# TongkunGuan/CCD

Hardware: AMD Instinct MI355X
Metric: images/sec (32x128 crops, 2 views) CCD-ViT-Small pretrain step (higher is better)
Workload: dtype bf16; 1 GPU; CCD_pretrain_vit_small bf16, bs=256/GPU, 2 views 32x128, out_dim=65536, drop_path 0.1, dataset-mask branch (pseudo-epoch 1), synthetic batch in HBM; global_batch=256, parallelism=dp1

## Files before the change

### ccd_amd/csrc/abi_impl.h

```cpp
#pragma once

#include "../../include/ccd_hip.h"
#include "kernels/common.h"
#include "kernels/gemm.h"
#include "kernels/gemm256.h"
#include "kernels/gemm_row384.h"
#include "kernels/mlp_fused.h"
#include "kernels/rowgemm.h"
#include "kernels/mlp_bwd.h"
#include "kernels/rowproj.h"
#include "kernels/attention_fwd.h"
#include "kernels/attention_probs.h"
#include "kernels/attention_bwd.h"
#include "kernels/attention_bwd1.h"
#include "kernels/gemm_tn384.h"
#include "kernels/layernorm.h"
#include "kernels/charmap.h"
#include "kernels/cluster.h"
#include "kernels/ssim.h"
#include "kernels/segmetric.h"
#include "kernels/textscore.h"
#include "kernels/ctc.h"
#include "kernels/ctc_beam.h"
#include "kernels/nrtr_beam.h"
// ... 959 lines not shown
    CCD_CHECK(ccd::aug_spatial_smem(height, width) <= 160 * 1024, CCD_ESHAPE);
    CCD_CHECK(std3[0] > 0.f && std3[1] > 0.f && std3[2] > 0.f, CCD_EINVAL);
    if (batch == 0) return CCD_OK;
    CCD_LAUNCH(ccd::augment_spatial_kernel, dim3(2 * batch), dim3(256), (int)ccd::aug_spatial_smem(height, width), stream, img, params,
               staged_ws, height, width, overlay, overlay_layers);
    CCD_LAUNCH(ccd::augment_views_kernel, dim3((height * width + 255) / 256, batch), dim3(256), 0, stream, img, staged_ws, theta,
               out, batch, height, width, mean3[0], mean3[1], mean3[2], 1.0f / std3[0], 1.0f / std3[1], 1.0f / std3[2], params, warp_maps,
               warp_count);
    return ccd_rt_last_error();
}
int ccd_warp_idmap(const uint8_t* src, const float* theta, int theta_stride, uint8_t* dst, int images, void* stream) {
    CCD_CHECK(src && theta && dst && images >= 0 && theta_stride >= 6, CCD_EINVAL);
    if (images == 0) return CCD_OK;
    CCD_LAUNCH(ccd::warp_idmap_kernel, dim3(ccd::CM_PIX / 256, images), dim3(256), 0, stream, src, theta, theta_stride,
               dst, images);
    return ccd_rt_last_error();
}
int ccd_region_stats(const uint8_t* idmap, uint8_t* tok_plane, float* tok_coef, uint8_t* present, int views,
                     void* stream) {
    CCD_CHECK(idmap && tok_plane && tok_coef && present && views >= 0, CCD_EINVAL);
    if (views == 0) return CCD_OK;
    CCD_LAUNCH(ccd::region_stats_kernel, dim3(views), dim3(256), 0, stream, idmap, tok_plane, tok_coef, present, views);
    return ccd_rt_last_error();
}
int ccd_select_scan(const uint8_t* present, int batch, int* nsel, int* offset, int* total, uint8_t* new_index,
                    void* stream) {
    CCD_CHECK(present && nsel && offset && total && new_index && batch > 0, CCD_EINVAL);
    CCD_LAUNCH(ccd::select_scan_kernel, dim3(1), dim3(256), 0, stream, present, batch, nsel, offset, total, new_index);
    return ccd_rt_last_error();
}
int ccd_region_pool_fwd(const ccd_bf16* feat, const uint8_t* tok_plane, const float* tok_coef, const int* nsel,
                        const int* offset, const int* total, ccd_bf16* rows, int batch, int E, void* stream) {
    CCD_CHECK(feat && tok_plane && tok_coef && nsel && offset && total && rows && batch > 0 && E > 0, CCD_EINVAL);
    const size_t smem = (size_t)ccd::CM_PLANES * E * 4;
    CCD_CHECK(smem <= 120 * 1024 && E % 2 == 0, CCD_ESHAPE);
    CCD_LAUNCH(ccd::region_pool_fwd_kernel, dim3(2 * batch), dim3(256), smem, stream, feat, tok_plane, tok_coef, nsel,
               offset, total, rows, batch, E);
    return ccd_rt_last_error();
}
int ccd_region_pool_bwd(const ccd_bf16* d_rows, const uint8_t* tok_plane, const float* tok_coef, const int* nsel,
                        const int* offset, const int* total, ccd_bf16* d_feat, int batch, int E, void* stream) {
    CCD_CHECK(d_rows && tok_plane && tok_coef && nsel && offset && total && d_feat && batch > 0 && E > 0, CCD_EINVAL);
    CCD_CHECK(E % 8 == 0, CCD_ESHAPE);
    CCD_LAUNCH(ccd::region_pool_bwd_kernel, dim3(2 * batch), dim3(256), 0, stream, d_rows, tok_plane, tok_coef, nsel,
               offset, total, d_feat, batch, E);
    return ccd_rt_last_error();
}
int ccd_idmap_to_planes(const uint8_t* idmap, float* planes, int images, void* stream) {
    CCD_CHECK(idmap && planes && images >= 0, CCD_EINVAL);
    if (images == 0) return CCD_OK;
    const long n = (long)images * ccd::CM_PLANES * ccd::CM_PIX;
    CCD_LAUNCH(ccd::idmap_to_planes_kernel, dim3((unsigned)((n + 255) / 256)), dim3(256), 0, stream, idmap, planes,
               (long)images);
    return ccd_rt_last_error();
}
int ccd_planes_to_idmap(const float* planes, uint8_t* idmap, int images, void* stream) {
    CCD_CHECK(idmap && planes && images >= 0, CCD_EINVAL);
    if (images == 0) return CCD_OK;
    const long n = (long)images * ccd::CM_PIX;
    CCD_LAUNCH(ccd::planes_to_idmap_kernel, dim3((unsigned)((n + 255) / 256)), dim3(256), 0, stream, planes, idmap,
               (long)images);
    return ccd_rt_last_error();
}

int ccd_dbscan_label(const float* mask, uint8_t* idmap, int images, void* stream) {
    CCD_CHECK(images >= 0, CCD_EINVAL);
    if (images == 0) return CCD_OK;
    CCD_CHECK(mask && idmap, CCD_EINVAL);
    CCD_LAUNCH(ccd::dbscan_label_kernel, dim3(images), dim3(256), 0, stream, mask, idmap, images);
    return ccd_rt_last_error();
}
int ccd_region_boxes(const float* mask, int* boxes, int* count, int images, void* stream) {
    CCD_CHECK(images >= 0, CCD_EINVAL);
    if (images == 0) return CCD_OK;
    CCD_CHECK(mask && boxes && count, CCD_EINVAL);
    CCD_LAUNCH(ccd::region_boxes_kernel, dim3(images), dim3(256), 0, stream, mask, boxes, count, images);
    return ccd_rt_last_error();
// ... 431 lines not shown
int ccd_nrtr_beam_reorder(ccd_bf16* cache, const int* parent, int layers, int batch, int beam, int positions, int D, int step, void* stream) {
    CCD_CHECK(layers >= 0 && batch >= 0 && step >= 0, CCD_EINVAL);
    CCD_CHECK(beam >= 1 && beam <= ccd::NRTR_MAX_BEAM && positions >= 1 && step < positions && D >= 8 && D % 8 == 0, CCD_ESHAPE);
    if (layers == 0 || batch == 0) return CCD_OK;
    CCD_CHECK(cache && parent && CCD_ALIGNED16(cache), CCD_EINVAL);
    const long total = (long)layers * batch * (step + 1) * (D / 4);
    CCD_CHECK((total + 255) / 256 <= 0x7fffffffL, CCD_ESHAPE);
    CCD_LAUNCH(ccd::nrtr_beam_reorder_kernel, dim3((unsigned)((total + 255) / 256)), dim3(256), 0, stream,
               reinterpret_cast<ccd::bf16_t*>(cache), parent, layers, batch, beam, positions, D, step, total);
    return ccd_rt_last_error();
}

int ccd_l2norm_fwd(const ccd_bf16* x, ccd_bf16* y, float* inv, int max_rows, const int* d_rows, int rows_mul, int D,
                   void* stream) {
    CCD_CHECK(x && y && inv && max_rows >= 0, CCD_EINVAL);
    if (max_rows == 0) return CCD_OK;
    CCD_CHECK(D > 0 && D <= 64 * ccd::HD_MAX_PER_LANE, CCD_ESHAPE);
    CCD_LAUNCH(ccd::l2norm_fwd_kernel, dim3((max_rows + 3) / 4), dim3(256), 0, stream, x, y, inv, max_rows, d_rows,
               rows_mul, D);
    return ccd_rt_last_error();
}
int ccd_l2norm_bwd(const ccd_bf16* x, const float* inv, const ccd_bf16* dy, ccd_bf16* dx, int max_rows,
                   const int* d_rows, int rows_mul, int D, void* stream) {
    CCD_CHECK(x && inv && dy && dx && max_rows >= 0, CCD_EINVAL);
    if (max_rows == 0) return CCD_OK;
    CCD_CHECK(D > 0 && D <= 64 * ccd::HD_MAX_PER_LANE, CCD_ESHAPE);
    CCD_LAUNCH(ccd::l2norm_bwd_kernel, dim3((max_rows + 3) / 4), dim3(256), 0, stream, x, inv, dy, dx, max_rows, d_rows,
               rows_mul, D);
    return ccd_rt_last_error();
}
int ccd_weightnorm_fwd(const float* v, const float* g, ccd_bf16* w, ccd_bf16* w_t, float* inv, int K, int D,
                       void* stream) {
    CCD_CHECK(v && g && w && inv && K > 0 && D > 0, CCD_EINVAL);
    const size_t smem = (size_t)ccd::WN_ROWS * (D + 1) * 4;
    CCD_CHECK(smem <= 128 * 1024 && D % 4 == 0 && D <= 256 * ccd::WN_MAX_V4 && K % 2 == 0, CCD_ESHAPE);
    CCD_LAUNCH(ccd::weightnorm_fwd_kernel, dim3((K + ccd::WN_ROWS - 1) / ccd::WN_ROWS), dim3(256), smem, stream, v, g, w, w_t, inv, K, D);
    return ccd_rt_last_error();
}
int ccd_weightnorm_bwd(const float* v, const float* g, const float* inv, const float* dw, float* dv, float* dg, int K,
                       int D, void* stream) {
    CCD_CHECK(v && g && inv && dw && dv && K > 0 && D > 0, CCD_EINVAL);
    CCD_LAUNCH(ccd::weightnorm_bwd_kernel, dim3((K + 3) / 4), dim3(256), 0, stream, v, g, inv, dw, dv, dg, K, D);
    return ccd_rt_last_error();
}

int ccd_dino_loss_fwd(const float* s_logits, const float* t_logits, const float* center, int K, const int* d_m,
                      int max_rows, float student_temp, float teacher_temp, float* stats, float* loss_out,
                      void* stream) {
    CCD_CHECK(s_logits && t_logits && center && d_m && stats && loss_out, CCD_EINVAL);
    CCD_CHECK(K > 0 && K % 4 == 0 && max_rows > 0 && student_temp > 0 && teacher_temp > 0, CCD_ESHAPE);
    CCD_LAUNCH(ccd::dino_loss_fwd_kernel, dim3(max_rows), dim3(256), 0, stream, s_logits, t_logits, center, K, d_m,
               max_rows, 1.0f / student_temp, 1.0f / teacher_temp, stats, loss_out);
    return ccd_rt_last_error();
}
int ccd_dino_loss_bwd(const float* s_logits, const float* t_logits, const float* center, int K, const int* d_m,
                      int max_rows, float student_temp, float teacher_temp, const float* stats, float grad_scale,
                      const float* d_grad_scale, ccd_bf16* d_logits, void* stream) {
    CCD_CHECK(s_logits && t_logits && center && d_m && stats && d_logits, CCD_EINVAL);
    CCD_CHECK(K > 0 && K % 4 == 0 && max_rows > 0 && student_temp > 0 && teacher_temp > 0, CCD_ESHAPE);
    CCD_LAUNCH(ccd::dino_loss_bwd_kernel, dim3(max_rows), dim3(256), 0, stream, s_logits, t_logits, center, K, d_m,
               max_rows, 1.0f / student_temp, 1.0f / teacher_temp, stats, grad_scale, d_grad_scale, d_logits);
    return ccd_rt_last_error();
}
static int ccd_head_loss_splits(int K) {
    if (K <= 0 || K % 512 != 0) return 0;
    const int chunks_total = K / 64;
    for (int cs = 64; cs >= 8; cs -= 8)
        if (chunks_total % cs == 0) return cs;
// ... 730 lines not shown
```

### ccd_amd/csrc/kernels/charmap.h

```cpp
#pragma once

namespace ccd {

constexpr int CM_H = 32, CM_W = 128, CM_PIX = CM_H * CM_W, CM_PLANES = 26, CM_MIN_AREA = 30;
constexpr unsigned char CM_BG = 255;

__device__ __forceinline__ void cm_components(int* label, int* changed) {
    const int t = threadIdx.x;
    for (;;) {
        if (t == 0) *changed = 0;
        __syncthreads();
        for (int i = t; i < CM_PIX; i += 256) {
            const int li = label[i];
            if (li < 0) continue;
            const int y = i >> 7, x = i & 127;
            int best = li;
#pragma unroll
            for (int dy = -1; dy <= 1; ++dy)
#pragma unroll
                for (int dx = -1; dx <= 1; ++dx) {
                    const int yy = y + dy, xx = x + dx;
                    if (yy < 0 || yy >= CM_H || xx < 0 || xx >= CM_W) continue;
                    const int ln = label[yy * CM_W + xx];
                    if (ln >= 0 && ln < best) best = ln;
// ... 181 lines not shown
                                                          unsigned char* __restrict__ new_index) {
    __shared__ int part[256];
    const int t = threadIdx.x;
    const int per = (batch + 255) / 256;
    int local = 0;
    for (int k = 0; k < per; ++k) {
        const int b = t * per + k;
        if (b >= batch) break;
        int c = 0;
        for (int j = 0; j < CM_PLANES; ++j) c += present[(long)b * CM_PLANES + j];
        c = c < 3 ? 3 : (c > 26 ? 26 : c);
        const int n = c + 1 < CM_PLANES ? c + 1 : CM_PLANES;
        nsel[b] = n;
        local += n;
        for (int j = 0; j < CM_PLANES; ++j) new_index[(long)b * CM_PLANES + j] = j <= c ? 1 : 0;
    }
    part[t] = local;
    __syncthreads();
    if (t == 0) {
        int run = 0;
        for (int k = 0; k < 256; ++k) { const int v = part[k]; part[k] = run; run += v; }
        total[0] = run;
    }
    __syncthreads();
    int run = part[t];
    for (int k = 0; k < per; ++k) {
        const int b = t * per + k;
        if (b >= batch) break;
        offset[b] = run;
        run += nsel[b];
    }
}

__global__ __launch_bounds__(256) void region_pool_fwd_kernel(const bf16_t* __restrict__ feat,
                                                              const unsigned char* __restrict__ tok_plane,
                                                              const float* __restrict__ tok_coef,
                                                              const int* __restrict__ nsel, const int* __restrict__ offset,
                                                              const int* __restrict__ total, bf16_t* __restrict__ rows,
                                                              int batch, int E) {
    float* acc = reinterpret_cast<float*>(dynamic_smem());
    __shared__ unsigned char s_plane[256 * 4];
    __shared__ float s_coef[256 * 4];
    const int view = blockIdx.x, b = view % batch, half = view / batch;
    const int t = threadIdx.x;
#pragma unroll
    for (int s = 0; s < 4; ++s) {
        s_plane[4 * t + s] = tok_plane[((long)view * 256 + t) * 4 + s];
        s_coef[4 * t + s] = tok_coef[((long)view * 256 + t) * 4 + s];
    }
    const int n = nsel[b];
    for (int i = t; i < n * E; i += 256) acc[i] = 0.0f;
    __syncthreads();
    const bf16_t* f = feat + (long)view * 256 * E;
    for (int e2 = t; 2 * e2 < E; e2 += 256) {
        for (int tok0 = 0; tok0 < 256; tok0 += 8) {
            unsigned wv[8];
#pragma unroll
            for (int u = 0; u < 8; ++u) wv[u] = *reinterpret_cast<const unsigned*>(f + (long)(tok0 + u) * E + 2 * e2);
#pragma unroll
            for (int u = 0; u < 8; ++u) {
                const int tok = tok0 + u;
                if (s_plane[4 * tok] == CM_BG) continue;
                const float x0 = bf_lo(wv[u]), x1 = bf_hi(wv[u]);
#pragma unroll
                for (int s = 0; s < 4; ++s) {
                    const int p = s_plane[4 * tok + s];
                    if (p < n) {
                        const float cf = s_coef[4 * tok + s];
                        acc[p * E + 2 * e2] += cf * x0;
                        acc[p * E + 2 * e2 + 1] += cf * x1;
                    }
                }
            }
        }
    }
    __syncthreads();
    bf16_t* out = rows + ((long)half * total[0] + offset[b]) * E;
    for (int i = t; i < n * E; i += 256) out[i] = f2bf(acc[i]);
}

__global__ __launch_bounds__(256) void region_pool_bwd_kernel(const bf16_t* __restrict__ d_rows,
                                                              const unsigned char* __restrict__ tok_plane,
                                                              const float* __restrict__ tok_coef,
                                                              const int* __restrict__ nsel, const int* __restrict__ offset,
                                                              const int* __restrict__ total, bf16_t* __restrict__ d_feat,
                                                              int batch, int E) {
    const int view = blockIdx.x, b = view % batch, half = view / batch;
    const int n = nsel[b];
    const bf16_t* base = d_rows + ((long)half * total[0] + offset[b]) * E;
    bf16_t* out = d_feat + (long)view * 256 * E;
    const int e8 = E >> 3;
    for (int i = threadIdx.x; i < 256 * e8; i += 256) {
        const int tok = i / e8, c = i % e8;
        float a[8] = {0.f, 0.f, 0.f, 0.f, 0.f, 0.f, 0.f, 0.f};
#pragma unroll
        for (int s = 0; s < 4; ++s) {
            const int p = tok_plane[((long)view * 256 + tok) * 4 + s];
            if (p < n) {
                const float coef = tok_coef[((long)view * 256 + tok) * 4 + s];
                float v[8];
                unpack8(*reinterpret_cast<const u32x4*>(base + (long)p * E + c * 8), v);
#pragma unroll
                for (int k = 0; k < 8; ++k) a[k] += v[k] * coef;
            }
        }
        *reinterpret_cast<u32x4*>(out + (long)tok * E + c * 8) = pack8(a);
    }
}

__global__ void idmap_to_planes_kernel(const unsigned char* __restrict__ idmap, float* __restrict__ planes, long images) {
    const long i = (long)blockIdx.x * blockDim.x + threadIdx.x;
    if (i >= images * CM_PLANES * CM_PIX) return;
    const long img = i / (CM_PLANES * CM_PIX);
    const int plane = (int)((i / CM_PIX) % CM_PLANES), pix = (int)(i % CM_PIX);
    planes[i] = idmap[img * CM_PIX + pix] == plane ? 1.0f : 0.0f;
}
__global__ void planes_to_idmap_kernel(const float* __restrict__ planes, unsigned char* __restrict__ idmap, long images) {
    const long i = (long)blockIdx.x * blockDim.x + threadIdx.x;
    if (i >= images * CM_PIX) return;
    const long img = i / CM_PIX;
    const int pix = (int)(i % CM_PIX);
    int id = CM_BG;
    for (int p = CM_PLANES - 1; p >= 0; --p)
        if (planes[(img * CM_PLANES + p) * CM_PIX + pix] > 0.0f) id = p;
    idmap[i] = (unsigned char)id;
}

}
```

### ccd_amd/csrc/kernels/embed.h

```cpp
#pragma once

namespace ccd {

constexpr int PE_PATCH = 4, PE_K = 48, PE_GW = 32, PE_GH = 8;

__global__ __launch_bounds__(128) void patch_embed_fwd_kernel(const float* __restrict__ img, const float* __restrict__ w,
                                                              const float* __restrict__ bias,
                                                              const float* __restrict__ pos, float* __restrict__ out,
                                                              int E) {
    __shared__ float px[3][PE_PATCH][PE_GW * PE_PATCH];
    const int view = blockIdx.x / PE_GH, py = blockIdx.x % PE_GH;
    const float* src = img + (long)view * 3 * 32 * 128;
    for (int i = threadIdx.x; i < 3 * 4 * 128; i += blockDim.x) {
        const int c = i / 512, r = (i / 128) % 4, x = i % 128;
        px[c][r][x] = src[(long)c * 4096 + (py * 4 + r) * 128 + x];
    }
    __syncthreads();
    for (int e = threadIdx.x; e < E; e += blockDim.x) {
        float wr[PE_K];
#pragma unroll
        for (int k = 0; k < PE_K; ++k) wr[k] = w[(long)e * PE_K + k];
        const float b = bias[e];
        for (int tx = 0; tx < PE_GW; ++tx) {
            float acc = 0.f;
// ... 152 lines not shown
#pragma unroll
                for (int k = 0; k < 8; ++k) acc[k] += v[k];
            }
        }
        for (; r < r1; r += rln) {
            float v[8];
            unpack8(*reinterpret_cast<const u32x4*>(x + (long)r * ld + col), v);
#pragma unroll
            for (int k = 0; k < 8; ++k) acc[k] += v[k];
        }
    }
#pragma unroll
    for (int k = 0; k < 8; ++k) red[threadIdx.x][k] = acc[k];
    __syncthreads();
    if ((int)threadIdx.x < 8 * cgn) {
        const int c_local = threadIdx.x, g = c_local >> 3, k = c_local & 7;
        const int c = blockIdx.x * cgn * 8 + c_local;
        if (c < N) {
            float s = 0.f;
            for (int j = 0; j < rln; ++j) s += red[j * cgn + g][k];
            atomicAdd(out + c, s);
        }
    }
}

struct MirrorDesc {
    const float* src;
    bf16_t* dst;
    bf16_t* dst_t;
    int rows, cols;
    int tile_begin;
};
constexpr int MIRROR_TILE = 64;
__global__ __launch_bounds__(256) void mirror_bf16_kernel(const MirrorDesc* __restrict__ descs, int ndesc) {
    __shared__ float tile[MIRROR_TILE][MIRROR_TILE + 1];
    int d = 0;
    while (d + 1 < ndesc && descs[d + 1].tile_begin <= (int)blockIdx.x) ++d;
    const MirrorDesc m = descs[d];
    const int tiles_c = (m.cols + MIRROR_TILE - 1) / MIRROR_TILE;
    const int tl = blockIdx.x - m.tile_begin, tr = tl / tiles_c, tc = tl % tiles_c;
    const int lx = threadIdx.x & 63, ly = threadIdx.x >> 6;
    for (int i = ly; i < MIRROR_TILE; i += 4) {
        const int r = tr * MIRROR_TILE + i, c = tc * MIRROR_TILE + lx;
        float v = 0.f;
        if (r < m.rows && c < m.cols) {
            v = m.src[(long)r * m.cols + c];
            if (m.dst) m.dst[(long)r * m.cols + c] = f2bf(v);
        }
        tile[i][lx] = v;
    }
    __syncthreads();
    if (m.dst_t) {
        const int rp = threadIdx.x & 31, cy = threadIdx.x >> 5;
        const int r = tr * MIRROR_TILE + 2 * rp;
        const bool pairs = (m.rows & 1) == 0;
        for (int i = cy; i < MIRROR_TILE; i += 8) {
            const int c = tc * MIRROR_TILE + i;
            if (c >= m.cols) break;
            bf16_t* o = m.dst_t + (long)c * m.rows + r;
            if (pairs && r + 1 < m.rows) *reinterpret_cast<unsigned*>(o) = pack_bf2(tile[2 * rp][i], tile[2 * rp + 1][i]);
            else {
                if (r < m.rows) o[0] = f2bf(tile[2 * rp][i]);
                if (r + 1 < m.rows) o[1] = f2bf(tile[2 * rp + 1][i]);
            }
        }
    }
}

__global__ __launch_bounds__(256) void scale_cast_rows_kernel(const float* __restrict__ src, bf16_t* __restrict__ dst,
                                                              const float* __restrict__ rowscale, int rows_per_sample,
                                                              long rows, int E) {
    const int e4 = E >> 2;
    const long i = (long)blockIdx.x * 256 + threadIdx.x;
    if (i >= rows * e4) return;
    const long r = i / e4;
    const int c = (int)(i % e4) * 4;
    const float s = rowscale ? rowscale[r / rows_per_sample] : 1.0f;
    const f32x4v v = *reinterpret_cast<const f32x4v*>(src + r * E + c);
    u32x2 o;
    o.x = pack_bf2(v.x * s, v.y * s);
    o.y = pack_bf2(v.z * s, v.w * s);
    *reinterpret_cast<u32x2*>(dst + r * E + c) = o;
}

__global__ void cast_bf16_kernel(const float* __restrict__ src, bf16_t* __restrict__ dst, long n) {
    const long i = ((long)blockIdx.x * blockDim.x + threadIdx.x) * 4;
    if (i + 3 < n) {
        const f32x4v v = *reinterpret_cast<const f32x4v*>(src + i);
        u32x2 o;
        o.x = pack_bf2(v.x, v.y);
        o.y = pack_bf2(v.z, v.w);
        *reinterpret_cast<u32x2*>(dst + i) = o;
    } else {
        for (long k = i; k < n; ++k) dst[k] = f2bf(src[k]);
    }
}

// ... 2 lines not shown
```

### ccd_amd/csrc/kernels/head.h

```cpp
#pragma once

namespace ccd {

constexpr int HD_MAX_PER_LANE = 8;

__global__ __launch_bounds__(256) void l2norm_fwd_kernel(const bf16_t* __restrict__ x, bf16_t* __restrict__ y,
                                                         float* __restrict__ inv_out, int max_rows,
                                                         const int* __restrict__ d_rows, int rows_mul, int D) {
    const int lane = threadIdx.x & 63;
    const int row = blockIdx.x * 4 + (threadIdx.x >> 6);
    const int rows = d_rows ? d_rows[0] * rows_mul : max_rows;
    if (row >= rows || row >= max_rows) return;
    float v[HD_MAX_PER_LANE];
    float s = 0.f;
#pragma unroll
    for (int i = 0; i < HD_MAX_PER_LANE; ++i) {
        const int c = lane + 64 * i;
        v[i] = c < D ? bf2f(x[(long)row * D + c]) : 0.f;
        s += v[i] * v[i];
    }
    const float nrm = sqrtf(wave_sum(s));
    const float inv = 1.0f / fmaxf(nrm, 1e-12f);
#pragma unroll
    for (int i = 0; i < HD_MAX_PER_LANE; ++i) {
// ... 2 lines not shown
    }
    if (lane == 0) inv_out[row] = inv;
}
__global__ __launch_bounds__(256) void l2norm_bwd_kernel(const bf16_t* __restrict__ x, const float* __restrict__ inv_in,
                                                         const bf16_t* __restrict__ dy, bf16_t* __restrict__ dx,
                                                         int max_rows, const int* __restrict__ d_rows, int rows_mul,
                                                         int D) {
    const int lane = threadIdx.x & 63;
    const int row = blockIdx.x * 4 + (threadIdx.x >> 6);
    const int rows = d_rows ? d_rows[0] * rows_mul : max_rows;
    if (row >= rows || row >= max_rows) return;
    const float inv = inv_in[row];
    float yv[HD_MAX_PER_LANE], dv[HD_MAX_PER_LANE];
    float dot = 0.f;
#pragma unroll
    for (int i = 0; i < HD_MAX_PER_LANE; ++i) {
        const int c = lane + 64 * i;
        yv[i] = c < D ? bf2f(x[(long)row * D + c]) * inv : 0.f;
        dv[i] = c < D ? bf2f(dy[(long)row * D + c]) : 0.f;
        dot += yv[i] * dv[i];
    }
    dot = wave_sum(dot);
#pragma unroll
    for (int i = 0; i < HD_MAX_PER_LANE; ++i) {
        const int c = lane + 64 * i;
        if (c < D) dx[(long)row * D + c] = f2bf(inv * (dv[i] - yv[i] * dot));
    }
}

constexpr int WN_ROWS = 64, WN_MAX_V4 = 4;
__global__ __launch_bounds__(256) void weightnorm_fwd_kernel(const float* __restrict__ v, const float* __restrict__ g,
                                                             bf16_t* __restrict__ w, bf16_t* __restrict__ w_t,
                                                             float* __restrict__ inv_out, int K, int D) {
    float* tile = reinterpret_cast<float*>(dynamic_smem());
    const int lane = threadIdx.x & 63, wv = threadIdx.x >> 6;
    const int k0 = blockIdx.x * WN_ROWS;
    const int d4 = D >> 2;
    for (int r = wv; r < WN_ROWS; r += 4) {
        const int k = k0 + r;
        if (k >= K) break;
        const f32x4v* row = reinterpret_cast<const f32x4v*>(v + (long)k * D);
        f32x4v x[WN_MAX_V4];
        float s = 0.f;
#pragma unroll
        for (int j = 0; j < WN_MAX_V4; ++j) {
            const int c4 = lane + 64 * j;
            x[j] = c4 < d4 ? row[c4] : f32x4v{0.f, 0.f, 0.f, 0.f};
            s += x[j].x * x[j].x + x[j].y * x[j].y + x[j].z * x[j].z + x[j].w * x[j].w;
        }
        const float inv = 1.0f / sqrtf(wave_sum(s));
        const float sc = g[k] * inv;
#pragma unroll
        for (int j = 0; j < WN_MAX_V4; ++j) {
            const int c4 = lane + 64 * j;
            if (c4 < d4) {
                const float a0 = x[j].x * sc, a1 = x[j].y * sc, a2 = x[j].z * sc, a3 = x[j].w * sc;
                u32x2 o;
                o.x = pack_bf2(a0, a1); o.y = pack_bf2(a2, a3);
                *reinterpret_cast<u32x2*>(w + (long)k * D + 4 * c4) = o;
                float* t = tile + r * (D + 1) + 4 * c4;
                t[0] = a0; t[1] = a1; t[2] = a2; t[3] = a3;
            }
        }
        if (lane == 0) inv_out[k] = inv;
    }
    __syncthreads();
    if (w_t) {
        const int kp = threadIdx.x & 31;
        for (int c = threadIdx.x >> 5; c < D; c += 8)
            if (k0 + 2 * kp + 1 < K)
                *reinterpret_cast<unsigned*>(w_t + (long)c * K + k0 + 2 * kp) =
                    pack_bf2(tile[(2 * kp) * (D + 1) + c], tile[(2 * kp + 1) * (D + 1) + c]);
    }
}
__global__ __launch_bounds__(256) void weightnorm_bwd_kernel(const float* __restrict__ v, const float* __restrict__ g,
                                                             const float* __restrict__ inv_in,
                                                             const float* __restrict__ dw, float* __restrict__ dv,
                                                             float* __restrict__ dg, int K, int D) {
    const int lane = threadIdx.x & 63;
    const int k = blockIdx.x * 4 + (threadIdx.x >> 6);
    if (k >= K) return;
    const float inv = inv_in[k], gk = g[k];
    float dot = 0.f;
    for (int c = lane; c < D; c += 64) dot += dw[(long)k * D + c] * v[(long)k * D + c] * inv;
    dot = wave_sum(dot);
    for (int c = lane; c < D; c += 64) {
        const float vh = v[(long)k * D + c] * inv;
        dv[(long)k * D + c] = gk * inv * (dw[(long)k * D + c] - vh * dot);
    }
    if (dg && lane == 0) dg[k] = dot;
}

}
```

### ccd_amd/engine.py

```python
from __future__ import annotations

import math

import os

import torch

from . import ops

BF16, F32 = torch.bfloat16, torch.float32


class VitSpec:
    def __init__(self, embed_dim, depth, heads, taps, patch=4, eps=1e-6, drop_path_rate=0.0):
        self.E, self.depth, self.heads, self.taps, self.patch, self.eps = embed_dim, depth, heads, tuple(taps), patch, eps
        self.dpr = [x.item() for x in torch.linspace(0, drop_path_rate, depth)]
        self._keep = {}

    def keep_probs(self, device):
        if device not in self._keep:
            self._keep[device] = torch.tensor([1.0 - d for d in self.dpr], dtype=F32, device=device)
        return self._keep[device]


# ... 414 lines not shown
    @staticmethod
    def backward(ctx, d_tokens, *d_taps):
        m = ctx.module
        cast = lambda t: None if t is None else t.contiguous().to(BF16)
        backbone_backward(m.arena, m.arena_prefix, m.spec, ctx.saved, cast(d_tokens), [cast(t) for t in d_taps],
                          m.resample, m.grad_ready_hook)
        ctx.saved = None
        return None, None, None, None


class Selection:

    def __init__(self, idmap, batch):
        self.idmap, self.batch = idmap, batch
        self.tok_plane, self.tok_coef, self.present = ops.region_stats(idmap)
        self.nsel, self.offset, self.total, self.new_index = ops.select_scan(self.present, batch)
        self.max_rows = 2 * 26 * batch
        self._m = None

    @property
    def M(self):
        if self._m is None:
            self._m = int(self.total.item())
        return self._m

    def dense(self):
        return ops.idmap_to_planes(self.idmap)


class RegionPoolFn(torch.autograd.Function):
    @staticmethod
    def forward(ctx, tokens, sel: Selection):
        E = tokens.shape[-1]
        rows = torch.zeros((sel.max_rows, E), dtype=BF16, device=tokens.device)
        ops.region_pool_fwd(tokens.contiguous(), sel.tok_plane, sel.tok_coef, sel.nsel, sel.offset, sel.total, rows,
                            sel.batch)
        ctx.sel, ctx.shape = sel, tokens.shape
        return rows

    @staticmethod
    def backward(ctx, d_rows):
        sel = ctx.sel
        d_feat = torch.empty(ctx.shape, dtype=BF16, device=d_rows.device)
        ops.region_pool_bwd(d_rows.contiguous().to(BF16), sel.tok_plane, sel.tok_coef, sel.nsel, sel.offset, sel.total,
                            d_feat, sel.batch)
        return d_feat, None


class LazyLogits:

    def __init__(self, zn, w, d_total, rows_mul):
        self.zn, self.w, self.d_total, self.rows_mul = zn, w, d_total, rows_mul
        self.stub = None
        self._tensor = None

    @property
    def shape(self):
        return torch.Size((self.zn.shape[0], self.w.shape[0]))

    @property
    def device(self):
        return self.zn.device

    def detach(self):
        return self

    def tensor(self):
# ... 210 lines not shown
```

### ccd_amd/ops.py

```python
from __future__ import annotations

import ctypes
import math

import numpy as np
import torch

from . import _lib

EPI_BF16, EPI_GELU, EPI_RESID, EPI_F32, EPI_ATOMIC, EPI_DGELU = range(6)
BF16, F32 = torch.bfloat16, torch.float32
_EPI_NAMES = ("bf16", "gelu", "resid", "f32", "atomic", "dgelu")


class KernelTimer:

    def __init__(self, only=None):
        self.records = []
        self.only = only

    def span(self, key, flops, nbytes=0.0):
        if self.only is not None and key not in self.only:
            return None
        e0, e1 = torch.cuda.Event(enable_timing=True), torch.cuda.Event(enable_timing=True)
# ... 443 lines not shown
    _call("ccd_augment_views", img, params, theta, out, staged, B, H, W, m3, s3, overlay, int(layers), warp_maps, int(maps))
    return out


def warp_idmap(src, theta):
    assert src.dtype == U8 and src.is_contiguous() and theta.dtype == F32 and theta.is_contiguous()
    out = torch.empty_like(src)
    _call("ccd_warp_idmap", src, theta, theta.stride(0), out, src.shape[0])
    return out


def region_stats(idmap):
    views = idmap.shape[0]
    dev = idmap.device
    tok_plane = torch.empty((views, 256, 4), dtype=U8, device=dev)
    tok_coef = torch.empty((views, 256, 4), dtype=F32, device=dev)
    present = torch.empty((views, 26), dtype=U8, device=dev)
    _call("ccd_region_stats", idmap, tok_plane, tok_coef, present, views)
    return tok_plane, tok_coef, present


def select_scan(present, batch):
    dev = present.device
    nsel = torch.empty(batch, dtype=I32, device=dev)
    offset = torch.empty(batch, dtype=I32, device=dev)
    total = torch.empty(1, dtype=I32, device=dev)
    new_index = torch.empty((batch, 26), dtype=U8, device=dev)
    _call("ccd_select_scan", present, batch, nsel, offset, total, new_index)
    return nsel, offset, total, new_index


def region_pool_fwd(feat, tok_plane, tok_coef, nsel, offset, total, rows, batch):
    E = feat.shape[-1]
    _call("ccd_region_pool_fwd", feat, tok_plane, tok_coef, nsel, offset, total, rows, batch, E)
    return rows


def region_pool_bwd(d_rows, tok_plane, tok_coef, nsel, offset, total, d_feat, batch):
    E = d_feat.shape[-1]
    _call("ccd_region_pool_bwd", d_rows, tok_plane, tok_coef, nsel, offset, total, d_feat, batch, E)
    return d_feat


def idmap_to_planes(idmap):
    out = torch.empty((idmap.shape[0], 26, 32, 128), dtype=F32, device=idmap.device)
    _call("ccd_idmap_to_planes", idmap, out, idmap.shape[0])
    return out


def planes_to_idmap(planes):
    planes = planes.contiguous().float()
    out = torch.empty((planes.shape[0], 32, 128), dtype=U8, device=planes.device)
    _call("ccd_planes_to_idmap", planes, out, planes.shape[0])
    return out


def dbscan_label(mask):
    assert mask.dtype == F32 and mask.is_contiguous() and tuple(mask.shape[1:]) == (32, 128)
    out = torch.empty(mask.shape, dtype=U8, device=mask.device)
    _call("ccd_dbscan_label", mask, out, mask.shape[0])
    return out


def region_boxes(mask):
    assert mask.dtype == F32 and mask.is_contiguous() and tuple(mask.shape[1:]) == (32, 128)
    boxes = torch.empty((mask.shape[0], 26, 4), dtype=I32, device=mask.device)
# ... 1307 lines not shown
```

Baseline: 5554 images/sec.

## Rework region pooling, weightnorm, and mirror kernels for parallelism and vectorized access

Region pool forward moves from one 256-thread block per view to many 64-thread blocks, each owning a channel slab. The new version double-buffers token chunks through LDS, zero-fills the unused output rows inside the kernel, and drops the separate torch.zeros memset. Region pool backward splits each view across four blocks and stages plane and coefficient data in shared memory. The weightnorm forward/backward and the fp32-to-bf16 mirror/transpose kernels switch to vectorized 128-bit loads and stores, with bf16 LDS tiles using swizzled or padded layouts. These changes target low occupancy and narrow memory accesses, at the cost of more complex indexing and a cap of 27 region planes per view in forward.

```diff
diff --git a/ccd_amd/csrc/abi_impl.h b/ccd_amd/csrc/abi_impl.h
--- a/ccd_amd/csrc/abi_impl.h
+++ b/ccd_amd/csrc/abi_impl.h
@@ -1015,17 +1015,20 @@
 int ccd_region_pool_fwd(const ccd_bf16* feat, const uint8_t* tok_plane, const float* tok_coef, const int* nsel,
                         const int* offset, const int* total, ccd_bf16* rows, int batch, int E, void* stream) {
     CCD_CHECK(feat && tok_plane && tok_coef && nsel && offset && total && rows && batch > 0 && E > 0, CCD_EINVAL);
-    const size_t smem = (size_t)ccd::CM_PLANES * E * 4;
-    CCD_CHECK(smem <= 120 * 1024 && E % 2 == 0, CCD_ESHAPE);
-    CCD_LAUNCH(ccd::region_pool_fwd_kernel, dim3(2 * batch), dim3(256), smem, stream, feat, tok_plane, tok_coef, nsel,
-               offset, total, rows, batch, E);
+    CCD_CHECK(E % 8 == 0, CCD_ESHAPE);
+    if (E % 128 == 0)
+        CCD_LAUNCH(ccd::region_pool_fwd_kernel<16>, dim3(2 * batch * (E / 128)), dim3(64), 0, stream, feat, tok_plane, tok_coef, nsel,
+                   offset, total, rows, batch, E);
+    else
+        CCD_LAUNCH(ccd::region_pool_fwd_kernel<8>, dim3(2 * batch * ((E + 63) / 64)), dim3(64), 0, stream, feat, tok_plane, tok_coef, nsel,
+                   offset, total, rows, batch, E);
     return ccd_rt_last_error();
 }
 int ccd_region_pool_bwd(const ccd_bf16* d_rows, const uint8_t* tok_plane, const float* tok_coef, const int* nsel,
                         const int* offset, const int* total, ccd_bf16* d_feat, int batch, int E, void* stream) {
     CCD_CHECK(d_rows && tok_plane && tok_coef && nsel && offset && total && d_feat && batch > 0 && E > 0, CCD_EINVAL);
     CCD_CHECK(E % 8 == 0, CCD_ESHAPE);
-    CCD_LAUNCH(ccd::region_pool_bwd_kernel, dim3(2 * batch), dim3(256), 0, stream, d_rows, tok_plane, tok_coef, nsel,
+    CCD_LAUNCH(ccd::region_pool_bwd_kernel, dim3(2 * batch * (256 / ccd::RPB_TOK)), dim3(256), 0, stream, d_rows, tok_plane, tok_coef, nsel,
                offset, total, d_feat, batch, E);
     return ccd_rt_last_error();
 }
@@ -1523,8 +1526,8 @@
 int ccd_weightnorm_fwd(const float* v, const float* g, ccd_bf16* w, ccd_bf16* w_t, float* inv, int K, int D,
                        void* stream) {
     CCD_CHECK(v && g && w && inv && K > 0 && D > 0, CCD_EINVAL);
-    const size_t smem = (size_t)ccd::WN_ROWS * (D + 1) * 4;
-    CCD_CHECK(smem <= 128 * 1024 && D % 4 == 0 && D <= 256 * ccd::WN_MAX_V4 && K % 2 == 0, CCD_ESHAPE);
+    const size_t smem = (size_t)ccd::WN_ROWS * (D + 2) * 2;
+    CCD_CHECK(smem <= 128 * 1024 && D % 4 == 0 && D <= 256 * ccd::WN_MAX_V4, CCD_ESHAPE);
     CCD_LAUNCH(ccd::weightnorm_fwd_kernel, dim3((K + ccd::WN_ROWS - 1) / ccd::WN_ROWS), dim3(256), smem, stream, v, g, w, w_t, inv, K, D);
     return ccd_rt_last_error();
 }
diff --git a/ccd_amd/csrc/kernels/charmap.h b/ccd_amd/csrc/kernels/charmap.h
--- a/ccd_amd/csrc/kernels/charmap.h
+++ b/ccd_amd/csrc/kernels/charmap.h
@@ -237,72 +237,120 @@
     }
 }
 
-__global__ __launch_bounds__(256) void region_pool_fwd_kernel(const bf16_t* __restrict__ feat,
-                                                              const unsigned char* __restrict__ tok_plane,
-                                                              const float* __restrict__ tok_coef,
-                                                              const int* __restrict__ nsel, const int* __restrict__ offset,
-                                                              const int* __restrict__ total, bf16_t* __restrict__ rows,
-                                                              int batch, int E) {
-    float* acc = reinterpret_cast<float*>(dynamic_smem());
-    __shared__ unsigned char s_plane[256 * 4];
-    __shared__ float s_coef[256 * 4];
-    const int view = blockIdx.x, b = view % batch, half = view / batch;
-    const int t = threadIdx.x;
-#pragma unroll
-    for (int s = 0; s < 4; ++s) {
-        s_plane[4 * t + s] = tok_plane[((long)view * 256 + t) * 4 + s];
-        s_coef[4 * t + s] = tok_coef[((long)view * 256 + t) * 4 + s];
-    }
-    const int n = nsel[b];
-    for (int i = t; i < n * E; i += 256) acc[i] = 0.0f;
-    __syncthreads();
-    const bf16_t* f = feat + (long)view * 256 * E;
-    for (int e2 = t; 2 * e2 < E; e2 += 256) {
-        for (int tok0 = 0; tok0 < 256; tok0 += 8) {
-            unsigned wv[8];
-#pragma unroll
-            for (int u = 0; u < 8; ++u) wv[u] = *reinterpret_cast<const unsigned*>(f + (long)(tok0 + u) * E + 2 * e2);
-#pragma unroll
-            for (int u = 0; u < 8; ++u) {
-                const int tok = tok0 + u;
-                if (s_plane[4 * tok] == CM_BG) continue;
-                const float x0 = bf_lo(wv[u]), x1 = bf_hi(wv[u]);
+constexpr int RP_CHUNK = 32, RP_MAXP = CM_PLANES + 1;
+template <int OCT>
+__global__ __launch_bounds__(64) void region_pool_fwd_kernel(const bf16_t* __restrict__ feat,
+                                                             const unsigned char* __restrict__ tok_plane,
+                                                             const float* __restrict__ tok_coef,
+                                                             const int* __restrict__ nsel, const int* __restrict__ offset,
+                                                             const int* __restrict__ total, bf16_t* __restrict__ rows,
+                                                             int batch, int E) {
+    constexpr int CLS = 64 / OCT, TPL = RP_CHUNK / CLS;
+    __shared__ f32x4v acc[RP_MAXP * 2 * OCT];
+    __shared__ u32x4 chunk[RP_CHUNK * OCT];
+    __shared__ u32x4 s_plane4[256 * 4 / 16];
+    __shared__ f32x4v c_coef[RP_CHUNK];
+    const unsigned* s_plane = reinterpret_cast<const unsigned*>(s_plane4);
+    const int nslab = (E + 8 * OCT - 1) / (8 * OCT);
+    const int view = blockIdx.x / nslab, slab = blockIdx.x % nslab, b = view % batch, half = view / batch;
+    const int lane = threadIdx.x, o = lane % OCT, k = lane / OCT;
+    const int ch = (slab * OCT + o) * 8;
+    const bool live = ch < E;
+    s_plane4[lane] = reinterpret_cast<const u32x4*>(tok_plane + (long)view * 1024)[lane];
+    const f32x4v* coef4 = reinterpret_cast<const f32x4v*>(tok_coef) + (long)view * 256;
+    f32x4v nxc = lane < RP_CHUNK ? coef4[lane] : f32x4v{0.f, 0.f, 0.f, 0.f};
+    int n = nsel[b];
+    n = n < RP_MAXP ? n : RP_MAXP;
+    for (int i = lane; i < n * 2 * OCT; i += 64) acc[i] = f32x4v{0.f, 0.f, 0.f, 0.f};
+    const bf16_t* f = feat + (long)view * 256 * E + ch;
+    u32x4 nxt[TPL];
+#pragma unroll
+    for (int u = 0; u < TPL; ++u) nxt[u] = live ? *reinterpret_cast<const u32x4*>(f + (long)(u * CLS + k) * E) : u32x4{0u, 0u, 0u, 0u};
+    for (int tok0 = 0; tok0 < 256; tok0 += RP_CHUNK) {
+        __syncthreads();
+#pragma unroll
+        for (int u = 0; u < TPL; ++u) chunk[(u * CLS + k) * OCT + o] = nxt[u];
+        if (lane < RP_CHUNK) c_coef[lane] = nxc;
+        __syncthreads();
+        if (tok0 + RP_CHUNK < 256) {
+#pragma unroll
+            for (int u = 0; u < TPL; ++u)
+                if (live) nxt[u] = *reinterpret_cast<const u32x4*>(f + (long)(tok0 + RP_CHUNK + u * CLS + k) * E);
+            if (lane < RP_CHUNK) nxc = coef4[tok0 + RP_CHUNK + lane];
+        }
+        for (int t4 = 0; t4 < RP_CHUNK; t4 += 4) {
+            const u32x4 pw = s_plane4[(tok0 + t4) >> 2];
+            const unsigned pl4[4] = {pw.x, pw.y, pw.z, pw.w};
+            u32x4 xw[4];
+            f32x4v cw[4];
+#pragma unroll
+            for (int u = 0; u < 4; ++u) { xw[u] = chunk[(t4 + u) * OCT + o]; cw[u] = c_coef[t4 + u]; }
+#pragma unroll
+            for (int u = 0; u < 4; ++u) {
+                const unsigned pl = pl4[u];
+                if ((pl & 255u) == CM_BG) continue;
+                float x[8];
+                unpack8(xw[u], x);
+                const f32x4v cf4 = cw[u];
+                const float cfs[4] = {cf4.x, cf4.y, cf4.z, cf4.w};
 #pragma unroll
                 for (int s = 0; s < 4; ++s) {
-                    const int p = s_plane[4 * tok + s];
-                    if (p < n) {
-                        const float cf = s_coef[4 * tok + s];
-                        acc[p * E + 2 * e2] += cf * x0;
-                        acc[p * E + 2 * e2 + 1] += cf * x1;
+                    const int p = (pl >> (8 * s)) & 255u;
+                    if (p < n && p % CLS == k) {
+                        const float cf = cfs[s];
+                        f32x4v a0 = acc[(2 * p) * OCT + o], a1 = acc[(2 * p + 1) * OCT + o];
+                        a0.x += cf * x[0]; a0.y += cf * x[1]; a0.z += cf * x[2]; a0.w += cf * x[3];
+                        a1.x += cf * x[4]; a1.y += cf * x[5]; a1.z += cf * x[6]; a1.w += cf * x[7];
+                        acc[(2 * p) * OCT + o] = a0; acc[(2 * p + 1) * OCT + o] = a1;
                     }
                 }
             }
         }
     }
     __syncthreads();
-    bf16_t* out = rows + ((long)half * total[0] + offset[b]) * E;
-    for (int i = t; i < n * E; i += 256) out[i] = f2bf(acc[i]);
-}
-
+    if (!live) return;
+    const int M = total[0];
+    bf16_t* out = rows + ((long)half * M + offset[b]) * E + ch;
+    for (int p = k; p < n; p += CLS) {
+        const f32x4v a0 = acc[(2 * p) * OCT + o], a1 = acc[(2 * p + 1) * OCT + o];
+        const float a[8] = {a0.x, a0.y, a0.z, a0.w, a1.x, a1.y, a1.z, a1.w};
+        *reinterpret_cast<u32x4*>(out + (long)p * E) = pack8(a);
+    }
+    for (long r = 2L * M + view * CLS + k; r < 2L * CM_PLANES * batch; r += 2L * batch * CLS)
+        *reinterpret_cast<u32x4*>(rows + r * E + ch) = u32x4{0u, 0u, 0u, 0u};
+}
+
+constexpr int RPB_TOK = 64;
 __global__ __launch_bounds__(256) void region_pool_bwd_kernel(const bf16_t* __restrict__ d_rows,
                                                               const unsigned char* __restrict__ tok_plane,
                                                               const float* __restrict__ tok_coef,
                                                               const int* __restrict__ nsel, const int* __restrict__ offset,
                                                               const int* __restrict__ total, bf16_t* __restrict__ d_feat,
                                                               int batch, int E) {
-    const int view = blockIdx.x, b = view % batch, half = view / batch;
+    __shared__ unsigned s_plane[RPB_TOK];
+    __shared__ f32x4v s_coef4[RPB_TOK];
+    constexpr int PARTS = 256 / RPB_TOK;
+    const int view = blockIdx.x / PARTS, tok0 = (blockIdx.x % PARTS) * RPB_TOK, b = view % batch, half = view / batch;
+    if (threadIdx.x < RPB_TOK) {
+        s_plane[threadIdx.x] = reinterpret_cast<const unsigned*>(tok_plane + ((long)view * 256 + tok0) * 4)[threadIdx.x];
+        s_coef4[threadIdx.x] = reinterpret_cast<const f32x4v*>(tok_coef + ((long)view * 256 + tok0) * 4)[threadIdx.x];
+    }
+    __syncthreads();
     const int n = nsel[b];
     const bf16_t* base = d_rows + ((long)half * total[0] + offset[b]) * E;
-    bf16_t* out = d_feat + (long)view * 256 * E;
+    bf16_t* out = d_feat + ((long)view * 256 + tok0) * E;
     const int e8 = E >> 3;
-    for (int i = threadIdx.x; i < 256 * e8; i += 256) {
+    for (int i = threadIdx.x; i < RPB_TOK * e8; i += 256) {
         const int tok = i / e8, c = i % e8;
+        const unsigned pl = s_plane[tok];
+        const f32x4v cf4 = s_coef4[tok];
+        const float cfs[4] = {cf4.x, cf4.y, cf4.z, cf4.w};
         float a[8] = {0.f, 0.f, 0.f, 0.f, 0.f, 0.f, 0.f, 0.f};
 #pragma unroll
         for (int s = 0; s < 4; ++s) {
-            const int p = tok_plane[((long)view * 256 + tok) * 4 + s];
+            const int p = (pl >> (8 * s)) & 255u;
             if (p < n) {
-                const float coef = tok_coef[((long)view * 256 + tok) * 4 + s];
+                const float coef = cfs[s];
                 float v[8];
                 unpack8(*reinterpret_cast<const u32x4*>(base + (long)p * E + c * 8), v);
 #pragma unroll
diff --git a/ccd_amd/csrc/kernels/embed.h b/ccd_amd/csrc/kernels/embed.h
--- a/ccd_amd/csrc/kernels/embed.h
+++ b/ccd_amd/csrc/kernels/embed.h
@@ -208,37 +208,65 @@
     int tile_begin;
 };
 constexpr int MIRROR_TILE = 64;
+__device__ __forceinline__ int mirror_lds_index(int c, int r) {
+    return c * MIRROR_TILE + ((((r >> 1) ^ ((c >> 3) << 2)) << 1) | (r & 1));
+}
 __global__ __launch_bounds__(256) void mirror_bf16_kernel(const MirrorDesc* __restrict__ descs, int ndesc) {
-    __shared__ float tile[MIRROR_TILE][MIRROR_TILE + 1];
+    __shared__ u32x4 tile4[MIRROR_TILE * MIRROR_TILE * 2 / 16];
+    bf16_t* tile = reinterpret_cast<bf16_t*>(tile4);
     int d = 0;
     while (d + 1 < ndesc && descs[d + 1].tile_begin <= (int)blockIdx.x) ++d;
     const MirrorDesc m = descs[d];
     const int tiles_c = (m.cols + MIRROR_TILE - 1) / MIRROR_TILE;
     const int tl = blockIdx.x - m.tile_begin, tr = tl / tiles_c, tc = tl % tiles_c;
+    const int r0 = tr * MIRROR_TILE, c0 = tc * MIRROR_TILE;
+    const unsigned long ptrs = reinterpret_cast<unsigned long>(m.src) | reinterpret_cast<unsigned long>(m.dst) |
+                               reinterpret_cast<unsigned long>(m.dst_t);
+    if (((m.rows | m.cols) & 7) == 0 && (ptrs & 15) == 0) {
+        const int cg = threadIdx.x & 7, rp = threadIdx.x >> 3;
+        const int r = r0 + 2 * rp, c = c0 + 8 * cg;
+        if (r < m.rows && c < m.cols) {
+            const f32x4v* s0 = reinterpret_cast<const f32x4v*>(m.src + (long)r * m.cols + c);
+            const f32x4v* s1 = reinterpret_cast<const f32x4v*>(m.src + (long)(r + 1) * m.cols + c);
+            const f32x4v a0 = s0[0], a1 = s0[1], b0 = s1[0], b1 = s1[1];
+            const float ra[8] = {a0.x, a0.y, a0.z, a0.w, a1.x, a1.y, a1.z, a1.w};
+            const float rb[8] = {b0.x, b0.y, b0.z, b0.w, b1.x, b1.y, b1.z, b1.w};
+            if (m.dst) {
+                *reinterpret_cast<u32x4*>(m.dst + (long)r * m.cols + c) = pack8(ra);
+                *reinterpret_cast<u32x4*>(m.dst + (long)(r + 1) * m.cols + c) = pack8(rb);
+            }
+            if (m.dst_t) {
+                unsigned* t32 = reinterpret_cast<unsigned*>(tile);
+#pragma unroll
+                for (int q = 0; q < 8; ++q) t32[mirror_lds_index(8 * cg + q, 2 * rp) >> 1] = pack_bf2(ra[q], rb[q]);
+            }
+        }
+        __syncthreads();
+        if (m.dst_t) {
+            const int rg = threadIdx.x & 7;
+#pragma unroll
+            for (int i = 0; i < 2; ++i) {
+                const int cl = (threadIdx.x >> 3) + 32 * i;
+                if (r0 + 8 * rg < m.rows && c0 + cl < m.cols)
+                    *reinterpret_cast<u32x4*>(m.dst_t + (long)(c0 + cl) * m.rows + r0 + 8 * rg) = tile4[mirror_lds_index(cl, 8 * rg) >> 3];
+            }
+        }
+        return;
+    }
     const int lx = threadIdx.x & 63, ly = threadIdx.x >> 6;
     for (int i = ly; i < MIRROR_TILE; i += 4) {
-        const int r = tr * MIRROR_TILE + i, c = tc * MIRROR_TILE + lx;
-        float v = 0.f;
+        const int r = r0 + i, c = c0 + lx;
         if (r < m.rows && c < m.cols) {
-            v = m.src[(long)r * m.cols + c];
-            if (m.dst) m.dst[(long)r * m.cols + c] = f2bf(v);
-        }
-        tile[i][lx] = v;
+            const bf16_t h = f2bf(m.src[(long)r * m.cols + c]);
+            if (m.dst) m.dst[(long)r * m.cols + c] = h;
+            tile[mirror_lds_index(lx, i)] = h;
+        }
     }
     __syncthreads();
     if (m.dst_t) {
-        const int rp = threadIdx.x & 31, cy = threadIdx.x >> 5;
-        const int r = tr * MIRROR_TILE + 2 * rp;
-        const bool pairs = (m.rows & 1) == 0;
-        for (int i = cy; i < MIRROR_TILE; i += 8) {
-            const int c = tc * MIRROR_TILE + i;
-            if (c >= m.cols) break;
-            bf16_t* o = m.dst_t + (long)c * m.rows + r;
-            if (pairs && r + 1 < m.rows) *reinterpret_cast<unsigned*>(o) = pack_bf2(tile[2 * rp][i], tile[2 * rp + 1][i]);
-            else {
-                if (r < m.rows) o[0] = f2bf(tile[2 * rp][i]);
-                if (r + 1 < m.rows) o[1] = f2bf(tile[2 * rp + 1][i]);
-            }
+        for (int i = ly; i < MIRROR_TILE; i += 4) {
+            const int r = r0 + lx, c = c0 + i;
+            if (r < m.rows && c < m.cols) m.dst_t[(long)c * m.rows + r] = tile[mirror_lds_index(i, lx)];
         }
     }
 }
diff --git a/ccd_amd/csrc/kernels/head.h b/ccd_amd/csrc/kernels/head.h
--- a/ccd_amd/csrc/kernels/head.h
+++ b/ccd_amd/csrc/kernels/head.h
@@ -58,61 +58,119 @@
 __global__ __launch_bounds__(256) void weightnorm_fwd_kernel(const float* __restrict__ v, const float* __restrict__ g,
                                                              bf16_t* __restrict__ w, bf16_t* __restrict__ w_t,
                                                              float* __restrict__ inv_out, int K, int D) {
-    float* tile = reinterpret_cast<float*>(dynamic_smem());
+    unsigned* tile = reinterpret_cast<unsigned*>(dynamic_smem());
     const int lane = threadIdx.x & 63, wv = threadIdx.x >> 6;
     const int k0 = blockIdx.x * WN_ROWS;
-    const int d4 = D >> 2;
-    for (int r = wv; r < WN_ROWS; r += 4) {
-        const int k = k0 + r;
-        if (k >= K) break;
-        const f32x4v* row = reinterpret_cast<const f32x4v*>(v + (long)k * D);
-        f32x4v x[WN_MAX_V4];
-        float s = 0.f;
+    const int d4 = D >> 2, pitch = (D >> 1) + 1;
+    for (int rb = wv; rb < WN_ROWS; rb += 16) {
+        f32x4v x[4][WN_MAX_V4];
 #pragma unroll
-        for (int j = 0; j < WN_MAX_V4; ++j) {
-            const int c4 = lane + 64 * j;
-            x[j] = c4 < d4 ? row[c4] : f32x4v{0.f, 0.f, 0.f, 0.f};
-            s += x[j].x * x[j].x + x[j].y * x[j].y + x[j].z * x[j].z + x[j].w * x[j].w;
-        }
-        const float inv = 1.0f / sqrtf(wave_sum(s));
-        const float sc = g[k] * inv;
+        for (int q = 0; q < 4; ++q) {
+            const f32x4v* row = reinterpret_cast<const f32x4v*>(v + (long)(k0 + rb + 4 * q) * D);
 #pragma unroll
-        for (int j = 0; j < WN_MAX_V4; ++j) {
-            const int c4 = lane + 64 * j;
-            if (c4 < d4) {
-                const float a0 = x[j].x * sc, a1 = x[j].y * sc, a2 = x[j].z * sc, a3 = x[j].w * sc;
-                u32x2 o;
-                o.x = pack_bf2(a0, a1); o.y = pack_bf2(a2, a3);
-                *reinterpret_cast<u32x2*>(w + (long)k * D + 4 * c4) = o;
-                float* t = tile + r * (D + 1) + 4 * c4;
-                t[0] = a0; t[1] = a1; t[2] = a2; t[3] = a3;
+            for (int j = 0; j < WN_MAX_V4; ++j) {
+                const int c4 = lane + 64 * j;
+                x[q][j] = (c4 < d4 && k0 + rb + 4 * q < K) ? row[c4] : f32x4v{0.f, 0.f, 0.f, 0.f};
             }
         }
-        if (lane == 0) inv_out[k] = inv;
+#pragma unroll
+        for (int q = 0; q < 4; ++q) {
+            const int r = rb + 4 * q, k = k0 + r;
+            if (k >= K) break;
+            float s = 0.f;
+#pragma unroll
+            for (int j = 0; j < WN_MAX_V4; ++j)
+                s += x[q][j].x * x[q][j].x + x[q][j].y * x[q][j].y + x[q][j].z * x[q][j].z + x[q][j].w * x[q][j].w;
+            const float inv = 1.0f / sqrtf(wave_sum(s));
+            const float sc = g[k] * inv;
+#pragma unroll
+            for (int j = 0; j < WN_MAX_V4; ++j) {
+                const int c4 = lane + 64 * j;
+                if (c4 < d4) {
+                    u32x2 o;
+                    o.x = pack_bf2(x[q][j].x * sc, x[q][j].y * sc); o.y = pack_bf2(x[q][j].z * sc, x[q][j].w * sc);
+                    *reinterpret_cast<u32x2*>(w + (long)k * D + 4 * c4) = o;
+                    tile[r * pitch + 2 * c4] = o.x; tile[r * pitch + 2 * c4 + 1] = o.y;
+                }
+            }
+            if (lane == 0) inv_out[k] = inv;
+        }
     }
     __syncthreads();
-    if (w_t) {
-        const int kp = threadIdx.x & 31;
-        for (int c = threadIdx.x >> 5; c < D; c += 8)
-            if (k0 + 2 * kp + 1 < K)
-                *reinterpret_cast<unsigned*>(w_t + (long)c * K + k0 + 2 * kp) =
-                    pack_bf2(tile[(2 * kp) * (D + 1) + c], tile[(2 * kp + 1) * (D + 1) + c]);
+    if (!w_t) return;
+    const bf16_t* t16 = reinterpret_cast<const bf16_t*>(tile);
+    if ((K & 7) == 0 && (reinterpret_cast<unsigned long>(w_t) & 15) == 0) {
+        const int kg = threadIdx.x & 7;
+        const int k = k0 + 8 * kg;
+        if (k < K) {
+            const bf16_t* t = t16 + (8 * kg) * (2 * pitch);
+            for (int c = threadIdx.x >> 3; c < D; c += 32) {
+                u32x4 o;
+                o.x = t[c] | ((unsigned)t[2 * pitch + c] << 16);
+                o.y = t[4 * pitch + c] | ((unsigned)t[6 * pitch + c] << 16);
+                o.z = t[8 * pitch + c] | ((unsigned)t[10 * pitch + c] << 16);
+                o.w = t[12 * pitch + c] | ((unsigned)t[14 * pitch + c] << 16);
+                *reinterpret_cast<u32x4*>(w_t + (long)c * K + k) = o;
+            }
+        }
+    } else {
+        const int r = threadIdx.x & 63;
+        if (k0 + r < K)
+            for (int c = threadIdx.x >> 6; c < D; c += 4) w_t[(long)c * K + k0 + r] = t16[r * (2 * pitch) + c];
     }
 }
 __global__ __launch_bounds__(256) void weightnorm_bwd_kernel(const float* __restrict__ v, const float* __restrict__ g,
                                                              const float* __restrict__ inv_in,
                                                              const float* __restrict__ dw, float* __restrict__ dv,
                                                              float* __restrict__ dg, int K, int D) {
-    const int lane = threadIdx.x & 63;
-    const int k = blockIdx.x * 4 + (threadIdx.x >> 6);
+    __shared__ f32x4v prod[4][64 * WN_MAX_V4];
+    const int lane = threadIdx.x & 63, wv = threadIdx.x >> 6;
+    const int k = blockIdx.x * 4 + wv;
     if (k >= K) return;
     const float inv = inv_in[k], gk = g[k];
+    const int d4 = D >> 2;
+    const unsigned long ptrs = reinterpret_cast<unsigned long>(v) | reinterpret_cast<unsigned long>(dw) | reinterpret_cast<unsigned long>(dv);
+    if ((D & 3) || d4 > 64 * WN_MAX_V4 || (ptrs & 15)) {
+        float dot = 0.f;
+        for (int c = lane; c < D; c += 64) dot += dw[(long)k * D + c] * v[(long)k * D + c] * inv;
+        dot = wave_sum(dot);
+        for (int c = lane; c < D; c += 64) {
+            const float vh = v[(long)k * D + c] * inv;
+            dv[(long)k * D + c] = gk * inv * (dw[(long)k * D + c] - vh * dot);
+        }
+        if (dg && lane == 0) dg[k] = dot;
+        return;
+    }
+    const f32x4v* vrow = reinterpret_cast<const f32x4v*>(v + (long)k * D);
+    const f32x4v* drow = reinterpret_cast<const f32x4v*>(dw + (long)k * D);
+    f32x4v x[WN_MAX_V4], y[WN_MAX_V4];
+#pragma unroll
+    for (int j = 0; j < WN_MAX_V4; ++j) {
+        const int c4 = lane + 64 * j;
+        if (c4 < d4) { x[j] = vrow[c4]; y[j] = drow[c4]; }
+    }
+#pragma unroll
+    for (int j = 0; j < WN_MAX_V4; ++j) {
+        const int c4 = lane + 64 * j;
+        if (c4 < d4) prod[wv][c4] = f32x4v{y[j].x * x[j].x, y[j].y * x[j].y, y[j].z * x[j].z, y[j].w * x[j].w};
+    }
+    wave_lds_fence();
+    const float* p = reinterpret_cast<const float*>(prod[wv]);
     float dot = 0.f;
-    for (int c = lane; c < D; c += 64) dot += dw[(long)k * D + c] * v[(long)k * D + c] * inv;
+    for (int c = lane; c < D; c += 64) dot += p[c] * inv;
     dot = wave_sum(dot);
-    for (int c = lane; c < D; c += 64) {
-        const float vh = v[(long)k * D + c] * inv;
-        dv[(long)k * D + c] = gk * inv * (dw[(long)k * D + c] - vh * dot);
+    f32x4v* orow = reinterpret_cast<f32x4v*>(dv + (long)k * D);
+#pragma unroll
+    for (int j = 0; j < WN_MAX_V4; ++j) {
+        const int c4 = lane + 64 * j;
+        if (c4 < d4) {
+            f32x4v o;
+            o.x = gk * inv * (y[j].x - x[j].x * inv * dot);
+            o.y = gk * inv * (y[j].y - x[j].y * inv * dot);
+            o.z = gk * inv * (y[j].z - x[j].z * inv * dot);
+            o.w = gk * inv * (y[j].w - x[j].w * inv * dot);
+            orow[c4] = o;
+        }
     }
     if (dg && lane == 0) dg[k] = dot;
 }
diff --git a/ccd_amd/engine.py b/ccd_amd/engine.py
--- a/ccd_amd/engine.py
+++ b/ccd_amd/engine.py
@@ -470,7 +470,7 @@
     @staticmethod
     def forward(ctx, tokens, sel: Selection):
         E = tokens.shape[-1]
-        rows = torch.zeros((sel.max_rows, E), dtype=BF16, device=tokens.device)
+        rows = torch.empty((sel.max_rows, E), dtype=BF16, device=tokens.device)
         ops.region_pool_fwd(tokens.contiguous(), sel.tok_plane, sel.tok_coef, sel.nsel, sel.offset, sel.total, rows,
                             sel.batch)
         ctx.sel, ctx.shape = sel, tokens.shape
diff --git a/ccd_amd/ops.py b/ccd_amd/ops.py
--- a/ccd_amd/ops.py
+++ b/ccd_amd/ops.py
@@ -499,6 +499,7 @@
 
 def region_pool_fwd(feat, tok_plane, tok_coef, nsel, offset, total, rows, batch):
     E = feat.shape[-1]
+    assert rows.shape[0] == 2 * 26 * batch and rows.shape[1] == E and rows.is_contiguous(), "rows must be [2 * 26 * batch, E]"
     _call("ccd_region_pool_fwd", feat, tok_plane, tok_coef, nsel, offset, total, rows, batch, E)
     return rows
 
```

Result: no change. 5569 images/sec (median of 6 runs) (+0.3%).
